# greatscottgadgets/libbtbb

Measured on AMD Instinct MI355X. Metric: Gbit/s raw bitstream scanned (LAP_ANY, err<=2), higher is better.
Workload: dtype u64; 1 GPU; promiscuous LAP_ANY scan, 4 GiB packed single-channel synthetic bitstream per GPU, max_ac_errors=2, sync word every 4096 symbols; symbols_per_gpu=34359738305, hits_per_gpu=6402406, parallelism=time-sharded x1 (btbbx_shard_plan: slices + 63-symbol halo), no collectives

## Files before the change

libbtbb_amd/csrc/packet.hip:

```cpp
#include <stdlib.h>
#include <string.h>
#include <atomic>
#include <type_traits>
#include "packet_launch.h"
#include "packet_core.h"

static uint32_t host_crc_byte(uint32_t crc, uint32_t byte)
{
	uint32_t x = (crc ^ byte) & 0xff;
	x ^= (x << 4) & 0xff;
	return ((crc >> 8) ^ (x << 8) ^ (x << 3) ^ (x >> 4)) & 0xffff;
}

int chain_upload(const HostTables &t)
{
	{
		int seen[16] = {0};
		for (int clk = 0; clk < 64; clk++) {
			uint32_t v = 0;
			for (int j = 0; j < 4; j++)
				v |= (uint32_t)t.whiten[(t.whiten_idx[clk] + 3 + j) % 127] << j;
			seen[v]++;
		}
		for (int v = 0; v < 16; v++)
// ... 197 lines not shown
{
	int rc = ctx_require();
	if (rc)
		return rc;
	hipLaunchKernelGGL(trials_state_kernel, dim3(64), dim3(64), 0, stream, d_sym, d_in, d_out, (TrialState *)d_state, d_trials);
	HIP_TRY(hipGetLastError());
	return BTBBX_OK;
}

int launch_trials_merge(const void *d_state, const btbbx_pkt_in *d_in, btbbx_pkt_out *d_out, uint8_t *d_pay,
			const TrialPlan *plan, hipStream_t stream)
{
	hipLaunchKernelGGL(trials_merge_kernel, dim3(1), dim3(64), 0, stream, (const TrialState *)d_state, d_in, d_out, d_pay,
			   *plan);
	HIP_TRY(hipGetLastError());
	return BTBBX_OK;
}

size_t trials_state_bytes() { return 64 * sizeof(TrialState); }

int launch_gather(const uint64_t *d_words, uint64_t n_words, uint64_t pitch_words, const btbbx_hit *d_hits, uint32_t n_packets,
		  const uint32_t *d_count, uint32_t max_length, uint64_t *d_packets, uint32_t *d_lengths, hipStream_t hip_stream)
{
	int rc = ctx_require();
	if (rc)
		return rc;
	if (!n_packets)
		return BTBBX_OK;
	hipLaunchKernelGGL(gather_kernel, dim3((n_packets + GATHER_PACKETS - 1) / GATHER_PACKETS), dim3(256), 0,
			   hip_stream, d_words, n_words, pitch_words, d_hits, n_packets, max_length, d_packets, d_lengths, d_count);
	HIP_TRY(hipGetLastError());
	return BTBBX_OK;
}

extern "C" int btbbx_gather_packets_device(const uint64_t *d_words, uint64_t n_words, uint64_t pitch_words,
					   const btbbx_hit *d_hits, uint32_t n_packets, uint32_t max_length,
					   uint64_t *d_packets, uint32_t *d_lengths, void *hip_stream)
{
	return launch_gather(d_words, n_words, pitch_words, d_hits, n_packets, nullptr, max_length, d_packets, d_lengths, (hipStream_t)hip_stream);
}

extern "C" int btbbx_trials_device(const uint64_t *d_packets, const btbbx_pkt_in *d_in, uint32_t n_packets,
				   btbbx_trial *d_trials, void *hip_stream)
{
	return launch_trials(d_packets, d_in, n_packets, nullptr, d_trials, (hipStream_t)hip_stream);
}

int launch_trials(const uint64_t *d_packets, const btbbx_pkt_in *d_in, uint32_t n_packets, const uint32_t *d_count,
		  btbbx_trial *d_trials, hipStream_t hip_stream)
{
	int rc = ctx_require();
	if (rc)
		return rc;
	if (!n_packets)
		return BTBBX_OK;
	if (n_packets <= 256) {
		hipLaunchKernelGGL(trials_wide_kernel, dim3(n_packets * 64), dim3(64), 0, (hipStream_t)hip_stream,
				   d_packets, d_in, n_packets, d_trials, d_count);
	} else {
		const uint32_t batches = (n_packets + TL_PACKETS - 1) / TL_PACKETS;
		const uint32_t resident = (uint32_t)ctx().num_cus * TL_WGS_PER_CU;
		hipLaunchKernelGGL(trials_linear_kernel, dim3(batches < resident ? batches : resident), dim3(TL_THREADS), 0,
				   (hipStream_t)hip_stream, d_packets, d_in, n_packets, d_trials, d_count);
	}
#ifdef TL_PROFILE
	if (n_packets > 256) {
		unsigned long long prof[16], tot = 0;
		(void)hipDeviceSynchronize();
		(void)hipMemcpyFromSymbol(prof, HIP_SYMBOL(g_tl_prof), sizeof(prof));
		for (int k = 0; k < 16; k++) tot += prof[k];
		fprintf(stderr, "trials profile:");
		for (int k = 0; k < 10; k++) fprintf(stderr, " %d:%.1f%%", k, 100.0 * (double)prof[k] / (double)(tot ? tot : 1));
		fprintf(stderr, "\n");
		static unsigned long long z[16];
		(void)hipMemcpyToSymbol(HIP_SYMBOL(g_tl_prof), z, sizeof(z));
	}
#endif
	HIP_TRY(hipGetLastError());
	return BTBBX_OK;
}

extern "C" int btbbx_uap_table_device(const uint64_t *d_packets, const btbbx_pkt_in *d_in, uint32_t n_packets,
				      uint16_t *d_table, void *hip_stream)
{
	int rc = ctx_require();
	if (rc)
		return rc;
	if (!n_packets)
		return BTBBX_OK;
	if ((uintptr_t)d_table & 15) {
		set_error("btbbx_uap_table_device: table must be 16-byte aligned");
		return BTBBX_E_ARG;
	}
	hipLaunchKernelGGL(uap_table_kernel, dim3((n_packets + 255) / 256), dim3(256), 0, (hipStream_t)hip_stream,
			   d_packets, d_in, n_packets, (uint4 *)d_table);
	HIP_TRY(hipGetLastError());
	return BTBBX_OK;
}

int launch_header_flags(const uint64_t *d_packets, const uint32_t *d_lengths, uint32_t n_packets, const uint32_t *d_count,
			uint8_t *d_present, hipStream_t stream)
{
	if (!n_packets)
		return BTBBX_OK;
	hipLaunchKernelGGL(header_flags_kernel, dim3((n_packets + 255) / 256), dim3(256), 0, stream, d_packets, d_lengths, n_packets, d_present, d_count);
	HIP_TRY(hipGetLastError());
	return BTBBX_OK;
}

int launch_decode_bytes(const uint8_t *d_sym, uint8_t *d_pay, const btbbx_pkt_in *d_in, btbbx_pkt_out *d_out,
			uint32_t mode, bool with_payload, hipStream_t stream)
{
	int rc = ctx_require();
	if (rc)
		return rc;
	hipLaunchKernelGGL(decode_bytes_kernel, dim3(1), dim3(64), 0, stream, d_sym, d_pay, d_in, d_out, mode,
			   with_payload ? 1 : 0);
	HIP_TRY(hipGetLastError());
	return BTBBX_OK;
}

int launch_decode(const uint64_t *d_packets, const btbbx_pkt_in *d_in, uint32_t n_packets,
		  btbbx_pkt_out *d_out, uint32_t mode, const TrialPlan *plan, hipStream_t stream)
{
	int rc = ctx_require();
	if (rc)
		return rc;
	if (!n_packets)
		return BTBBX_OK;
	TrialPlan p = {0, 0, 0};
	if (plan)
		p = *plan;
	if (mode & DEC_TRIALS) {
		if (mode != DEC_TRIALS || n_packets != 1) {
			set_error("decode: trial replay is a one-packet mode");
			return BTBBX_E_ARG;
		}
		hipLaunchKernelGGL(replay_kernel, dim3(1), dim3(64), 0, stream, d_packets, d_in, d_out, p);
		HIP_TRY(hipGetLastError());
		return BTBBX_OK;
	}
	hipLaunchKernelGGL(decode_kernel, dim3((n_packets + 63) / 64), dim3(64), 0, stream,
			   d_packets, d_in, n_packets, d_out, mode);
	HIP_TRY(hipGetLastError());
	return BTBBX_OK;
}

extern "C" int btbbx_decode_device(const uint64_t *d_packets, const btbbx_pkt_in *d_in, uint32_t n_packets,
				   btbbx_pkt_out *d_out, void *hip_stream)
{
	return launch_decode(d_packets, d_in, n_packets, d_out, DEC_HEADER | DEC_PAYLOAD, nullptr, (hipStream_t)hip_stream);
}

static int decode_hits_list_alloc(size_t bytes, hipStream_t stream, void **block)
{
	static std::atomic<uint64_t> pool_ready{0}, pool_absent{0};
	*block = nullptr;
	int dev = 0;
	HIP_TRY(hipGetDevice(&dev));
	const bool tracked = dev >= 0 && dev < 64;
	if (tracked && ((pool_absent.load() >> dev) & 1))
		return BTBBX_OK;
	if (tracked && !((pool_ready.load() >> dev) & 1)) {
		hipMemPool_t pool;
		uint64_t keep = UINT64_MAX;
		if (hipDeviceGetDefaultMemPool(&pool, dev) != hipSuccess ||
		    hipMemPoolSetAttribute(pool, hipMemPoolAttrReleaseThreshold, &keep) != hipSuccess) {
			(void)hipGetLastError();
			pool_absent.fetch_or(1ULL << dev);
			return BTBBX_OK;
		}
		pool_ready.fetch_or(1ULL << dev);
	}
	if (hipMallocAsync(block, bytes, stream) != hipSuccess) {
		(void)hipGetLastError();
		*block = nullptr;
	}
	return BTBBX_OK;
}

static int launch_decode_hits(const uint64_t *d_words, uint64_t n_words, uint64_t pitch_words, const btbbx_hit *d_hits,
			      const btbbx_pkt_in *d_in, uint32_t n_packets, const uint32_t *d_count, uint32_t max_length,
			      btbbx_pkt_out *d_out, uint32_t *d_lengths, const btbbx_pkt_in &one_in, uint32_t clk_div, hipStream_t stream)
{
	const uint32_t groups = (uint32_t)(((uint64_t)n_packets + 255) / 256);
	void *block;
	const int rc = decode_hits_list_alloc((size_t)groups * 4 * 64 * sizeof(uint4), stream, &block);
	if (rc)
		return rc;
	hipLaunchKernelGGL(decode_hits_kernel, dim3(groups), dim3(256), 0, stream, d_words, n_words, pitch_words, d_hits, d_in, n_packets,
			   d_count, max_length, d_out, d_lengths, DEC_HEADER | DEC_PAYLOAD, one_in, clk_div, (uint4 *)block);
	hipError_t e = hipGetLastError();
	if (block) {
		const hipError_t f = hipFreeAsync(block, stream);
		if (e == hipSuccess)
			e = f;
	}
	HIP_TRY(e);
	return BTBBX_OK;
}

extern "C" int btbbx_decode_hits_device(const uint64_t *d_words, uint64_t n_words, uint64_t pitch_words,
					const btbbx_hit *d_hits, const btbbx_pkt_in *d_in, uint32_t n_packets,
					uint32_t max_length, btbbx_pkt_out *d_out, uint32_t *d_lengths, void *hip_stream)
{
	int rc = ctx_require();
	if (rc)
		return rc;
	if (!n_packets)
		return BTBBX_OK;
	if (!d_words || !d_hits || !d_in || !d_out) {
		set_error("btbbx_decode_hits_device: null pointer");
		return BTBBX_E_ARG;
	}
	return launch_decode_hits(d_words, n_words, pitch_words, d_hits, d_in, n_packets, nullptr, max_length, d_out, d_lengths, btbbx_pkt_in{}, 1u,
				  (hipStream_t)hip_stream);
}

extern "C" int btbbx_decode_hits_counted_device(const uint64_t *d_words, uint64_t n_words, uint64_t pitch_words,
						const btbbx_hit *d_hits, const btbbx_pkt_in *d_in, const uint32_t *d_count,
						uint32_t cap, uint32_t max_length, btbbx_pkt_out *d_out, uint32_t *d_lengths,
						void *hip_stream)
{
	int rc = ctx_require();
	if (rc)
		return rc;
	if (!cap)
		return BTBBX_OK;
	if (!d_words || !d_hits || !d_in || !d_out || !d_count) {
		set_error("btbbx_decode_hits_counted_device: null pointer");
		return BTBBX_E_ARG;
	}
	rc = launch_decode_hits(d_words, n_words, pitch_words, d_hits, d_in, cap, d_count, max_length, d_out, d_lengths, btbbx_pkt_in{}, 1u,
				(hipStream_t)hip_stream);
	if (rc)
		return rc;
#ifdef DH_PROFILE
	{
		unsigned long long prof[8], total = 0;
		HIP_TRY(hipDeviceSynchronize());
		HIP_TRY(hipMemcpyFromSymbol(prof, HIP_SYMBOL(g_dh_prof), sizeof(prof)));
		for (int k = 0; k < 8; k++) total += prof[k];
		fprintf(stderr, "decode_hits profile (%% of wave time): loads %.1f type %.1f staging %.1f head-load %.1f present %.1f header %.1f payload %.1f store %.1f; s_memtime ticks per wave %.0f\n",
			100.0 * prof[0] / total, 100.0 * prof[1] / total, 100.0 * prof[2] / total, 100.0 * prof[3] / total,
			100.0 * prof[4] / total, 100.0 * prof[5] / total, 100.0 * prof[6] / total, 100.0 * prof[7] / total,
			(double)total / ((cap + 63) / 64));
		unsigned long long zero[8] = {0, 0, 0, 0, 0, 0, 0, 0};
		HIP_TRY(hipMemcpyToSymbol(HIP_SYMBOL(g_dh_prof), zero, sizeof(zero)));
	}
#endif
	return BTBBX_OK;
}

extern "C" int btbbx_decode_hits_piconet_phase_device(const uint64_t *d_words, uint64_t n_words, uint64_t pitch_words,
						      const btbbx_hit *d_hits, const uint32_t *d_count, uint32_t cap,
						      const btbbx_pkt_in *entry, uint32_t clk_div, uint32_t clk_phase, uint32_t max_length,
						      btbbx_pkt_out *d_out, uint32_t *d_lengths, void *hip_stream)
{
	int rc = ctx_require();
	if (rc)
		return rc;
	if (!cap)
		return BTBBX_OK;
	if (!d_words || !d_hits || !entry || !d_out || !clk_div || clk_phase >= clk_div) {
		set_error("btbbx_decode_hits_piconet_device: null pointer, clk_div = 0 or clk_phase >= clk_div");
		return BTBBX_E_ARG;
	}
	btbbx_pkt_in one = *entry;
	one.length = clk_phase;
	return launch_decode_hits(d_words, n_words, pitch_words, d_hits, nullptr, cap, d_count, max_length, d_out, d_lengths, one, clk_div,
				  (hipStream_t)hip_stream);
}

extern "C" int btbbx_decode_hits_piconet_device(const uint64_t *d_words, uint64_t n_words, uint64_t pitch_words,
						const btbbx_hit *d_hits, const uint32_t *d_count, uint32_t cap,
						const btbbx_pkt_in *entry, uint32_t clk_div, uint32_t max_length,
						btbbx_pkt_out *d_out, uint32_t *d_lengths, void *hip_stream)
{
	return btbbx_decode_hits_piconet_phase_device(d_words, n_words, pitch_words, d_hits, d_count, cap, entry, clk_div, 0, max_length,
						      d_out, d_lengths, hip_stream);
}
```

libbtbb_amd/csrc/packet_core.h:

```cpp
#pragma once
#include "defer_entry.h"

__constant__ ChainTables g_chain;

struct __attribute__((aligned(16))) ChainLds {
	uint32_t wh32[128];
	uint16_t crc[256];
	uint16_t crc_z[3][256];
	uint8_t  par23[1024];
	int8_t   fix23[32];
	uint16_t fixm23[32];
	uint8_t  whiten_idx[64];
	uint16_t adv32[2][256];
};
__device__ __attribute__((aligned(16))) ChainLds g_chain_lds_image;

#define LIN_MAXLEN 344
__device__ __attribute__((aligned(16))) uint16_t g_lin[LIN_MAXLEN * 16];
__device__ __attribute__((aligned(16))) uint16_t g_advw[7 * 2 * 256];
__device__ __attribute__((aligned(16))) uint16_t g_adv64inv[64 * 16];
__device__ __attribute__((aligned(16))) uint16_t g_adv64fwd[64 * 16];

#define F_WHITENED    (1u << 0)
#define F_CLK6_VALID  (1u << 4)
// ... 15 lines not shown
	const uint32_t *d = reinterpret_cast<const uint32_t *>(w);
	const uint32_t i = pos >> 5;
	const uint32_t v = __builtin_amdgcn_alignbit(d[i + 1], d[i], pos & 31);
	return n == 32 ? v : v & ((1u << n) - 1);
}

__device__ __forceinline__ uint64_t wh_bits_const(uint32_t idx, uint32_t n)
{
	uint32_t i = idx >> 6, s = idx & 63;
	uint64_t v = g_chain.whiten2[i] >> s;
	if (s + n > 64)
		v |= g_chain.whiten2[i + 1] << (64 - s);
	return n == 64 ? v : v & ((1ULL << n) - 1);
}

__device__ __forceinline__ uint32_t wh_start_const(uint32_t clock, uint32_t skip)
{
	return (g_chain.whiten_idx[clock & 63] + skip) % 127u;
}

__shared__ ChainLds g_lds;

__device__ __forceinline__ uint64_t wh_bits(uint32_t idx, uint32_t n)
{
	uint64_t v = g_lds.wh32[idx];
	if (n > 32) {
		const uint32_t j = idx + 32;
		v |= (uint64_t)g_lds.wh32[j >= 127 ? j - 127 : j] << 32;
	}
	return n == 64 ? v : v & ((1ULL << n) - 1);
}

__device__ __forceinline__ uint32_t wh_start(uint32_t clock, uint32_t skip)
{
	return (g_lds.whiten_idx[clock & 63] + skip) % 127u;
}

__device__ __forceinline__ uint32_t rev8(uint32_t b) { return __brev(b) >> 24; }

__device__ __forceinline__ uint32_t crc_byte_calc(uint32_t crc, uint32_t byte)
{
	uint32_t x = (crc ^ byte) & 0xff;
	x ^= (x << 4) & 0xff;
	return ((crc >> 8) ^ (x << 8) ^ (x << 3) ^ (x >> 4)) & 0xffff;
}
__device__ __forceinline__ uint32_t crc_byte(uint32_t crc, uint32_t byte)
{
	return (crc >> 8) ^ g_lds.crc[(crc ^ byte) & 0xff];
}

__device__ __forceinline__ uint32_t crc_word(uint32_t crc, uint32_t w)
{
	const uint32_t x = crc ^ w;
	return g_lds.crc_z[2][x & 0xff] ^ g_lds.crc_z[1][(x >> 8) & 0xff] ^ g_lds.crc_z[0][(w >> 16) & 0xff] ^ g_lds.crc[w >> 24];
}

__device__ __forceinline__ uint32_t crc_seed(uint32_t uap) { return rev8(uap & 0xff) << 8; }

__device__ __forceinline__ uint32_t uap_from_hec(uint32_t data, uint32_t hec)
{
#pragma unroll
	for (int i = 9; i >= 0; i--) {
		if (hec & 0x80)
			hec ^= 0x65;
		hec = ((hec << 1) | (((hec >> 7) ^ (data >> i)) & 1)) & 0xff;
	}
	return rev8(hec);
}

__device__ __forceinline__ uint32_t fec13(uint64_t v, uint32_t n, uint32_t &disagree)
{
	const uint64_t M = 0x9249249249249249ULL;
	uint64_t a = v & M, b = (v >> 1) & M, c = (v >> 2) & M;
	uint64_t maj = (a & b) | (b & c) | (c & a);
	uint64_t dis = (a ^ b) | (b ^ c) | (c ^ a);
	if (n < 21) {
		uint64_t keep = (1ULL << (3 * n)) - 1;
		maj &= keep;
		dis &= keep;
	}
	disagree = __popcll(dis);
	uint64_t x = maj;
	x = (x | x >> 2) & 0x30c30c30c30c30c3ULL;
	x = (x | x >> 4) & 0xf00f00f00f00f00fULL;
	x = (x | x >> 8) & 0x00ff0000ff0000ffULL;
	x = (x | x >> 16) & 0xffff00000000ffffULL;
	x = (x | x >> 32) & 0xffffffffULL;
	return (uint32_t)x;
}

__device__ __forceinline__ bool fec23_block(uint32_t blk, uint32_t &data)
{
	data = blk & 0x3ff;
	uint32_t diff = (blk >> 10) ^ g_lds.par23[data];
	int fix = g_lds.fix23[diff & 31];
	if (fix == -2)
		return false;
	if (fix >= 0)
		data ^= 1u << fix;
	return true;
}

__device__ void chain_lds_init()
{
	static_assert(sizeof(ChainLds) % 16 == 0, "the image is copied 16 bytes at a time");
	const uint4 *src = reinterpret_cast<const uint4 *>(&g_chain_lds_image);
	uint4 *dst = reinterpret_cast<uint4 *>(&g_lds);
	for (uint32_t i = threadIdx.x; i < sizeof(ChainLds) / 16; i += blockDim.x)
		dst[i] = src[i];
	__syncthreads();
}


struct OutRef {
	uint64_t *g = nullptr;
	uint32_t l = 0;
	__device__ OutRef() {}
	__device__ OutRef(uint64_t *p) : g(p) {}
	__device__ __forceinline__ static OutRef lds(uint32_t byte_address) { OutRef r; r.l = byte_address + 1; return r; }
	__device__ __forceinline__ uint64_t ld(uint32_t k) const
	{
		if (l)
			return *reinterpret_cast<const __attribute__((address_space(3))) uint64_t *>(l - 1 + 8u * k);
		return g[k];
	}
	__device__ __forceinline__ void st(uint32_t k, uint64_t v) const
	{
		if (l)
			*reinterpret_cast<__attribute__((address_space(3))) uint64_t *>(l - 1 + 8u * k) = v;
		else
			g[k] = v;
	}
};
struct PState {
	const uint64_t *w;
	uint32_t sh = 0;
	uint32_t wlimit = 0;
	uint32_t staged = 0;
	uint32_t stage_off = 0;
	bool direct = false;
	bool has_pre = false;
	uint32_t pre_hdr = 0, pre_dis = 0;
	int length;
	uint32_t flags;
	uint32_t uap, type;
	uint32_t lt_addr, hdr_flags, hec, header18;
	int plen;
	int phl;
	uint32_t ph16;
	uint32_t ph_written;
	uint32_t llid, flow;
	OutRef out;
	bool spoiled = false;
	uint4 *def_slot = nullptr;
	uint32_t def_pkt8 = 0;
	uint32_t def_nbits = 0;
	uint32_t written;
	uint32_t dirty;
	uint32_t ph_mask;
};
#define D_UT    1u
#define D_PLEN  2u
#define D_PHL   4u
#define D_LF    8u

__device__ __forceinline__ void pstate_enter(PState &s, const btbbx_pkt_in &pi)
{
	s.flags = pi.flags;
	s.uap = pi.uap;
	s.type = pi.type;
	s.llid = pi.llid;
	s.flow = pi.flow;
}
__device__ __forceinline__ void pstate_from_head(PState &s, int plen, int phl, uint32_t ph16, uint32_t lt_addr, uint32_t hdr_flags,
						 uint32_t hec, uint32_t header18)
{
	s.plen = plen;
	s.phl = phl;
	s.ph16 = ph16;
	s.ph_written = 0;
	s.dirty = 0;
	s.ph_mask = 0;
	s.lt_addr = lt_addr; s.hdr_flags = hdr_flags; s.hec = hec; s.header18 = header18;
	s.written = 0;
}
__device__ __forceinline__ void pstate_from_head(PState &s, const btbbx_pkt_out *o)
{
	pstate_from_head(s, o->payload_length, o->payload_header_length, (uint32_t)o->payload_header, o->lt_addr, o->hdr_flags, o->hec, o->header_packed);
}
__device__ __forceinline__ void pstate_blank_out(PState &s) { pstate_from_head(s, 0, 0, 0, 0, 0, 0, 0); }

__device__ __forceinline__ uint64_t s_bits(const PState &s, uint32_t pos, uint32_t n)
{
	if (!s.direct)
		return pk_bits(s.w, pos, n);
	if ((int)pos >= s.length)
		return 0;
	const uint32_t q = pos + s.sh, i = q >> 6, sft = q & 63;
	auto word = [&](uint32_t k) -> uint64_t {
		if (k < s.staged)
			return *reinterpret_cast<const __attribute__((address_space(3))) uint64_t *>(s.stage_off + 8u * k);
		return k < s.wlimit ? ((const __attribute__((address_space(1))) uint64_t *)(uintptr_t)s.w)[k] : 0ULL;
	};
	uint64_t v = word(i) >> sft;
	if (sft + n > 64)
		v |= word(i + 1) << (64 - sft);
	const uint32_t have = (uint32_t)s.length - pos;
	const uint32_t keep = n < have ? n : have;
	return keep == 64 ? v : v & ((1ULL << keep) - 1);
}

template <bool WRITE>
struct Sink {
	uint64_t acc = 0;
	uint32_t nacc = 0;
	uint32_t crc;
	uint64_t oacc = 0;
	uint32_t onacc = 0, oword = 0;
	OutRef out;
	__device__ Sink(uint32_t seed, OutRef o) : crc(seed), out(o) {}
	__device__ __forceinline__ void push(uint64_t bits, uint32_t n)
	{
		if (n == 32 && nacc == 0) {
			crc = crc_word(crc, (uint32_t)bits);
		} else {
			acc |= bits << nacc;
			nacc += n;
			while (nacc >= 8) {
				crc = crc_byte(crc, (uint32_t)acc & 0xff);
				acc >>= 8;
				nacc -= 8;
			}
		}
		if (WRITE) {
			oacc |= bits << onacc;
			onacc += n;
			if (onacc >= 64) {
				out.st(oword++, oacc);
				onacc -= 64;
				oacc = onacc ? bits >> (n - onacc) : 0;
			}
		}
	}
	__device__ __forceinline__ void flush()
	{
		if (WRITE && onacc) {
			uint64_t keep = ~0ULL << onacc;
			out.st(oword, (out.ld(oword) & keep) | oacc);
		}
	}
};

__device__ __forceinline__ bool whitened(const PState &s) { return s.flags & F_WHITENED; }

__device__ __forceinline__ uint64_t wh(const PState &s, uint32_t idx, uint32_t n)
{
	return whitened(s) ? wh_bits(idx, n) : 0ULL;
}

__device__ __forceinline__ uint32_t fec23_blocks4(const PState &s, uint32_t pos, uint32_t count, uint32_t (&data)[4])
{
	uint32_t blk[4], diff[4];
	const uint64_t sym60 = s_bits(s, pos, 60);
#pragma unroll
	for (int j = 0; j < 4; j++)
		blk[j] = (uint32_t)j < count ? (uint32_t)(sym60 >> (15 * j)) & 0x7fff : 0;
#pragma unroll
	for (int j = 0; j < 4; j++) {
		data[j] = blk[j] & 0x3ff;
		diff[j] = (blk[j] >> 10) ^ g_lds.par23[data[j]];
	}
	uint32_t ok = 0;
#pragma unroll
	for (int j = 0; j < 4; j++) {
		const int fix = g_lds.fix23[diff[j] & 31];
		if (fix >= 0)
			data[j] ^= 1u << fix;
		if (fix != -2)
			ok |= 1u << j;
	}
	return ok;
}

__device__ __forceinline__ bool fec23_ok(const PState &s, uint32_t pos, uint32_t nblocks)
{
	for (uint32_t k = 0; k < nblocks; k += 4) {
		uint32_t d[4];
		const uint32_t cnt = nblocks - k < 4 ? nblocks - k : 4;
		if ((fec23_blocks4(s, pos + 15 * k, cnt, d) & ((1u << cnt) - 1)) != (1u << cnt) - 1)
			return false;
	}
	return true;
}

__device__ __forceinline__ void defer_payload(PState &s, uint32_t clock, uint32_t nbits, uint32_t kind)
{
	const uint32_t ext = kind == DHL_DH ? nbits : kind == DHL_EV5 ? 8u : 15u * ((nbits + 9u) / 10u);
	const uint32_t nw = (s.sh + 122u + ext + 63u) >> 6;
	const uint64_t a = DEFER_PACK_A((uintptr_t)s.w, nw < s.wlimit ? nw : s.wlimit, s.sh);
	const uint64_t b = DEFER_PACK_B(s.def_pkt8, (uint32_t)s.length, nbits, kind, (s.flags & 1u) ? 1u : 0u, wh_start(clock, 18), s.uap & 0xffu);
	*s.def_slot = make_uint4((uint32_t)a, (uint32_t)(a >> 32), (uint32_t)b, (uint32_t)(b >> 32));
	s.def_nbits = nbits;
}

template <bool WRITE>
struct SinkW : Sink<WRITE> {
	__device__ SinkW(uint32_t seed, OutRef o) : Sink<WRITE>(seed, o) {}
	__device__ __forceinline__ void push(uint64_t bits, uint32_t n)
	{
		this->acc |= bits << this->nacc;
		this->nacc += n;
		if (this->nacc >= 32) {
			this->crc = crc_word(this->crc, (uint32_t)this->acc);
			this->acc >>= 32;
			this->nacc -= 32;
		}
		if (WRITE) {
			this->oacc |= bits << this->onacc;
			this->onacc += n;
			if (this->onacc >= 64) {
				this->out.st(this->oword++, this->oacc);
				this->onacc -= 64;
				this->oacc = this->onacc ? bits >> (n - this->onacc) : 0;
			}
		}
	}
	__device__ __forceinline__ void finish()
	{
		while (this->nacc >= 8) {
			this->crc = crc_byte(this->crc, (uint32_t)this->acc & 0xff);
			this->acc >>= 8;
			this->nacc -= 8;
		}
	}
};
template <bool WRITE>
__device__ __forceinline__ int do_fhs(PState &s, uint32_t clock)
{
	int size = s.length - 122;
	s.plen = 20;
	s.dirty |= D_PLEN;
	if (size < 240)
		return 1;
	uint64_t corr[3] = {0, 0, 0};
#pragma unroll
	for (uint32_t k = 0; k < 16; k += 4) {
		uint32_t d4[4];
		const uint32_t ok = fec23_blocks4(s, 122 + 15 * k, 4, d4);
#pragma unroll
		for (uint32_t j = 0; j < 4; j++) {
			if (!((ok >> j) & 1))
				return 0;
			const uint32_t d = d4[j], bit = 10 * (k + j);
			corr[bit >> 6] |= (uint64_t)d << (bit & 63);
			if ((bit & 63) > 54)
				corr[(bit >> 6) + 1] |= (uint64_t)d >> (64 - (bit & 63));
		}
	}
	int rv = 0;
	uint32_t c = clock;
	for (int attempt = 0; attempt < 33; attempt++) {
		if (attempt)
			c = 31 + attempt;
		uint32_t idx = wh_start(c, 18);
		uint32_t crc = crc_seed(s.uap);
		uint64_t pl[3];
		for (int i = 0; i < 3; i++) {
			uint32_t n = i < 2 ? 64 : 32;
			pl[i] = corr[i] ^ wh(s, idx, n);
			idx = (idx + n) % 127u;
			for (uint32_t b = 0; b < n; b += 32)
				crc = crc_word(crc, (uint32_t)(pl[i] >> b));
		}
		if (WRITE) {
			s.out.st(0, pl[0]);
			s.out.st(1, pl[1]);
			s.out.st(2, (s.out.ld(2) & ~0xffffffffULL) | pl[2]);
			if (s.written < 160) s.written = 160;
		}
		if (crc == 0) {
			rv = 1000;
			break;
		}
	}
	return rv;
}

template <bool WRITE>
__device__ __forceinline__ bool do_payload_header(PState &s, uint32_t pos, uint32_t clock, int header_bytes, int size, bool fec)
{
	uint32_t hbits = header_bytes == 2 ? 16 : 8;
	if (size < (int)hbits)
		return false;
	uint32_t raw;
	if (fec) {
		if (size < (header_bytes == 2 ? 30 : 15))
			return false;
		uint32_t d0, d1 = 0;
		if (!fec23_block((uint32_t)s_bits(s, pos, 15), d0))
			return false;
		if (header_bytes == 2 && !fec23_block((uint32_t)s_bits(s, pos + 15, 15), d1))
			return false;
		raw = (d0 | (d1 << 10)) & ((1u << hbits) - 1);
	} else {
		raw = (uint32_t)s_bits(s, pos, hbits);
	}
	uint32_t ph = raw ^ (uint32_t)wh(s, wh_start(clock, 18), hbits);
	s.ph16 = (s.ph16 & ~((1u << hbits) - 1)) | ph;
	s.ph_mask |= (1u << hbits) - 1;
	s.dirty |= D_PLEN | D_LF | D_PHL;
	if (s.ph_written < hbits) s.ph_written = hbits;
	int plen = header_bytes == 2 ? (int)((s.ph16 >> 3) & 0x3ff) + 4 : (int)((s.ph16 >> 3) & 0x1f) + 3;
	int cap;
	switch (s.type) {
	case 3:  cap = 20;  break;
	case 4:  cap = 30;  break;
	case 8:  cap = 12;  break;
	case 10: cap = 125; break;
	case 11: cap = 187; break;
	case 14: cap = 228; break;
	case 15: cap = 343; break;
	default: cap = 0;   break;
	}
	s.plen = plen < cap ? plen : cap;
	s.llid = s.ph16 & 3;
	s.flow = (s.ph16 >> 2) & 1;
	s.phl = header_bytes;
	return true;
}

template <bool WRITE>
__device__ __forceinline__ int do_DM(PState &s, uint32_t clock)
{
	uint32_t pos = 122;
	int size = s.length - 122;
	int header_bytes = 2, max_length;
	switch (s.type) {
	case 8:  pos += 80; size -= 80; header_bytes = 1; max_length = 12; break;
	case 3:  header_bytes = 1; max_length = 20; break;
	case 10: max_length = 125; break;
	case 14: max_length = 228; break;
	default: return 0;
	}
	if (!do_payload_header<WRITE>(s, pos, clock, header_bytes, size, true))
		return 0;
	if (s.plen > max_length)
		return 1;
	int nbits = s.plen * 8;
	if (nbits > size)
		return 1;
	uint32_t nblocks = (nbits + 9) / 10;
	if (WRITE && s.def_slot && !s.out.l && nbits > DHL_MIN_BITS) {
		defer_payload(s, clock, (uint32_t)nbits, DHL_DM);
		return 2;
// ... 274 lines not shown
```

libbtbb_amd/csrc/packet_stream.h:

```cpp
#pragma once


#ifdef DH_PROFILE
__device__ unsigned long long g_dh_prof[8];
#define DH_MARK(k) do { uint64_t now_; __builtin_amdgcn_sched_barrier(0); asm volatile("s_waitcnt vmcnt(0) lgkmcnt(0)\n\ts_memtime %0\n\ts_waitcnt lgkmcnt(0)" : "=s"(now_) : : "memory"); \
	__builtin_amdgcn_sched_barrier(0); dh_acc[k] += (uint32_t)(now_ - dh_t); dh_t = now_; } while (0)
#define DH_PARAMS , uint32_t *dh_acc, uint64_t &dh_t
#define DH_PASS , dh_acc, dh_t
#else
#define DH_MARK(k) do { } while (0)
#define DH_PARAMS
#define DH_PASS
#endif
__device__ __forceinline__ void decode_view(PState &s, const btbbx_pkt_in &pi, btbbx_pkt_out *o, uint32_t mode,
					    OutRef pay_out, uint64_t *head_out, const uint64_t *head_in DH_PARAMS)
{
	pstate_enter(s, pi);
	static_assert(offsetof(btbbx_pkt_out, payload) == 40 && offsetof(btbbx_pkt_out, payload_header) == 32, "head of btbbx_pkt_out");
	union Head {
		uint64_t q[5];
		struct {
			int32_t header_rv, payload_rv, payload_length, payload_header_length;
			uint32_t flags, header_packed;
			uint8_t header_present, type, lt_addr, hdr_flags, hec, llid, flow, uap;
// ... 509 lines not shown
					w0 = src[i0];
				if (i1 < p_nw)
					w1 = src[i1];
			}
		}
	};
	uint64_t nw0, nw1;
	request(0, nw0, nw1);
#pragma unroll 1
	for (uint32_t r = 0; r < rounds; r++) {
		const uint32_t e = r * R + grp;
		const bool has = e < n_ev;
		uint64_t pa = 0, pb = 0;
		if (has) {
			pa = lst[DHL_LIST + 2 * (first + e)];
			pb = lst[DHL_LIST + 2 * (first + e) + 1];
		}
		const uint32_t p_sh = DEFER_SH(pa);
		const uint32_t p_pkt = DEFER_PKT(pb), nbits = DEFER_NBITS(pb);
		const uint32_t kind = DEFER_KIND(pb), p_widx = DEFER_WIDX(pb), p_uap = DEFER_UAP(pb);
		const bool p_wht = DEFER_WHITENED(pb), is4 = has && kind == DHL_EV4;
		const uint32_t nblocks = nbits / 10u;
		const uint64_t w0 = nw0, w1 = nw1;
		const uint32_t sft = (p_sh + 122u) & 63u;
		const uint32_t low8 = (uint32_t)(sft ? (w0 >> sft) | (w1 << (64u - sft)) : w0) & 0xffu;
		const uint32_t first8 = (uint32_t)__shfl((int)low8, (int)gbase);
		uint64_t word = (uint64_t)(first8 * 0x01010101u) | (uint64_t)(first8 * 0x01010101u) << 32;
		uint32_t first_fail = nblocks;
		if (__ballot(is4)) {
			stg[2 * gbase + sub] = w0;
			stg[2 * gbase + G + sub] = w1;
			__builtin_amdgcn_fence(__ATOMIC_ACQ_REL, "wavefront");
			__builtin_amdgcn_wave_barrier();
			for (uint32_t n0 = 0; ; n0 += G) {
				const uint32_t n = n0 + sub;
				const bool on = is4 && 4u * n < nblocks;
				if (!__ballot(on))
					break;
				const uint32_t left = nblocks - 4u * n, have = on ? (left < 4u ? left : 4u) : 0u;
				const uint32_t q = p_sh + 122u + 60u * n, i = 4u * gbase + (on ? q >> 5 : 0u);
				const uint32_t v0 = stg32[i], v1 = stg32[i + 1], v2 = stg32[i + 2];
				const uint64_t vm = (1ULL << (15u * have)) - 1;
				const uint32_t x0 = __builtin_amdgcn_alignbit(v1, v0, q & 31u) & (uint32_t)vm;
				const uint32_t x1 = __builtin_amdgcn_alignbit(v2, v1, q & 31u) & (uint32_t)(vm >> 32);
				const uint32_t b2 = __builtin_amdgcn_alignbit(x1, x0, 30);
				uint32_t d0 = x0 & 0x3ffu, d1 = (x0 >> 15) & 0x3ffu, d2 = b2 & 0x3ffu, d3 = (x1 >> 13) & 0x3ffu;
				const uint32_t m0 = g_lds.fixm23[((x0 >> 10) & 31u) ^ g_lds.par23[d0]], m1 = g_lds.fixm23[((x0 >> 25) & 31u) ^ g_lds.par23[d1]];
				const uint32_t m2 = g_lds.fixm23[((b2 >> 10) & 31u) ^ g_lds.par23[d2]], m3 = g_lds.fixm23[((x1 >> 23) & 31u) ^ g_lds.par23[d3]];
				const uint32_t bad = (m0 >> 15) | (m1 >> 15) << 1 | (m2 >> 15) << 2 | (m3 >> 15) << 3;
				d0 ^= m0 & 0x3ffu;
				d1 ^= m1 & 0x3ffu;
				d2 ^= m2 & 0x3ffu;
				d3 ^= m3 & 0x3ffu;
				if (on) {
					const uint32_t byte = 5u * n, d = 2u * DHL_PB + 2u * gbase + (byte >> 2);
					const uint64_t v = ((uint64_t)(d3 >> 2) << 32 | (d0 | d1 << 10 | d2 << 20 | d3 << 30)) << (8u * (byte & 3u));
					__hip_atomic_fetch_or(lst32 + d, (uint32_t)v, __ATOMIC_RELAXED, __HIP_MEMORY_SCOPE_WAVEFRONT);
					__hip_atomic_fetch_or(lst32 + d + 1, (uint32_t)(v >> 32), __ATOMIC_RELAXED, __HIP_MEMORY_SCOPE_WAVEFRONT);
				}
				const uint64_t gm = (__ballot(bad != 0) >> gbase) & gmask;
				const uint32_t gl = gm ? (uint32_t)__builtin_ctzll(gm) : 0u;
				const uint32_t gb = (uint32_t)__shfl((int)bad, (int)(gbase + gl));
				if (gm && first_fail == nblocks)
					first_fail = 4u * (n0 + gl) + (uint32_t)__builtin_ctz(gb | 16u);
			}
			__builtin_amdgcn_fence(__ATOMIC_ACQ_REL, "wavefront");
			__builtin_amdgcn_wave_barrier();
			if (is4)
				word = lst[DHL_PB + lane];
			lst[DHL_PB + lane] = 0;
		}
		if (r + 1 < rounds)
			request(r + 1, nw0, nw1);
		const uint32_t T = nbits >> 6;
		const bool active = has && 64u * sub < nbits;
		uint64_t out = 0;
		if (active) {
			uint32_t idx = p_widx + wh_lane;
			idx = idx >= 127u ? idx - 127u : idx;
			out = word ^ (p_wht ? wh_bits(idx, 64) : 0ULL);
			if (sub == T)
				out &= (1ULL << (nbits & 63u)) - 1;
		}
		uint32_t reg;
		{
			const uint64_t cw = out ^ (sub == 0 ? (uint64_t)crc_seed(p_uap) : 0ULL);
			const uint32_t reg0 = crc_word(crc_word(0, (uint32_t)cw), (uint32_t)(cw >> 32));
			const uint32_t q = apply_columns(rinv, reg0);
			uint32_t x = q, t;
			t = (uint32_t)__builtin_amdgcn_mov_dpp((int)x, 0x111, 0xf, 0xf, true); x ^= sub >= 1 ? t : 0u;
			t = (uint32_t)__builtin_amdgcn_mov_dpp((int)x, 0x112, 0xf, 0xf, true); x ^= sub >= 2 ? t : 0u;
			t = (uint32_t)__builtin_amdgcn_mov_dpp((int)x, 0x114, 0xf, 0xf, true); x ^= sub >= 4 ? t : 0u;
			if (logg > 3) {
				t = (uint32_t)__builtin_amdgcn_mov_dpp((int)x, 0x118, 0xf, 0xf, true); x ^= sub >= 8 ? t : 0u;
			}
			if (logg > 4) {
				t = (uint32_t)__shfl((int)x, (int)(gbase + 15));
				x ^= sub >= 16 ? t : 0u;
			}
			reg = apply_columns(rfwd, x ^ q);
		}
		const uint32_t ok_blocks = first_fail < nblocks ? first_fail : nblocks;
		const uint32_t hi = is4 ? (ok_blocks ? 5u * (ok_blocks - 1u) / 4u : 0u) : (nbits >> 3) - 1u, lo = is4 ? 2u : 3u;
		uint32_t zero = 0;
#pragma unroll
		for (int i = 0; i < 8; i++) {
			uint32_t byte = (uint32_t)(out >> (8 * i)) & 0xffu;
			if (i == 1 && sub == 0)
				byte ^= crc_seed(p_uap) >> 8;
			reg = crc_byte(reg, byte);
			const uint32_t L = 8u * sub + (uint32_t)i + 1u;
			if (reg == 0 && L >= lo && L <= hi)
				zero |= 1u << i;
		}
		const uint64_t hm = (__ballot(has && zero != 0) >> gbase) & gmask;
		const uint32_t hl = hm ? (uint32_t)__builtin_ctzll(hm) : 0u;
		const uint32_t hz = (uint32_t)__shfl((int)zero, (int)(gbase + hl));
		const uint32_t L_hit = hm ? 8u * hl + (uint32_t)__builtin_ctz(hz | 0x100u) + 1u : 0u;
		if (has) {
			uint32_t plen, wbits;
			int rv;
			if (is4) {
				if (L_hit) {
					rv = 10; plen = L_hit; wbits = 10u * ((8u * L_hit + 9u) / 10u + 1u);
				} else {
					plen = hi + 1u; wbits = 10u * ok_blocks;
					rv = ok_blocks == 98u ? 2 : first_fail < nblocks && first_fail < 3u ? 0 : 1;
				}
			} else {
				const uint32_t bytes = nbits >> 3;
				if (L_hit) {
					rv = 10; plen = L_hit; wbits = 8u * (L_hit + 1u);
				} else {
					plen = bytes; wbits = nbits; rv = bytes == 182u ? 2 : 1;
				}
			}
			const uint32_t wT = wbits >> 6, wrem = wbits & 63u;
			if (64u * sub < wbits) {
				uint64_t v = out;
				if (sub == wT) {
					const uint64_t wm = (1ULL << wrem) - 1;
					v = (out & wm) | (outs[p_pkt].payload[sub] & ~wm);
				}
				outs[p_pkt].payload[sub] = v;
			}
			if (sub == 0) {
				outs[p_pkt].payload_length = (int32_t)plen;
				outs[p_pkt].payload_rv = rv;
			}
		}
	}
}

__device__ __forceinline__ void long_wave(dhl_u64_t *stg, dhl_u64_t *lst, const uint4 *slots, uint64_t dmask, btbbx_pkt_out *outs, uint32_t lane)
{
	const bool mine = (dmask >> lane) & 1;
	uint4 e = make_uint4(0, 0, 0, 0);
	if (mine)
		e = slots[lane];
	const bool ev = mine && DEFER_KIND_HI(e.w) >= DHL_EV4;
	const uint64_t ev_mask = __ballot(ev), dh_mask = dmask & ~ev_mask;
	const uint32_t n_dh = (uint32_t)__popcll(dh_mask), n_ev = (uint32_t)__popcll(ev_mask);
	const uint32_t own_words = mine ? (DEFER_NBITS_LO(e.z) + 63u) >> 6 : 0u;
	if (mine) {
		const uint64_t among = ev ? ev_mask : dh_mask;
		const uint32_t rank = (ev ? n_dh : 0u) + __builtin_amdgcn_mbcnt_hi((uint32_t)(among >> 32), __builtin_amdgcn_mbcnt_lo((uint32_t)among, 0u));
		lst[DHL_LIST + 2 * rank] = (uint64_t)e.x | (uint64_t)e.y << 32;
		lst[DHL_LIST + 2 * rank + 1] = (uint64_t)e.z | (uint64_t)e.w << 32;
	}
	if (n_dh) {
		const uint32_t w = ev ? 0u : own_words;
		if (__ballot(mine && !ev && DEFER_KIND_HI(e.w) == DHL_DM)) {
			const uint32_t logg = __ballot(w > 32) ? 5u : __ballot(w > 16) ? 4u : 3u;
			long_payloads(stg, lst, n_dh, logg, outs, lane);
		} else {
			dh_payloads(lst, n_dh, __ballot(w > 24) ? 4u : 3u, outs, lane);
		}
	}
	if (n_ev) {
		const uint32_t w = ev ? own_words : 0u;
		const uint32_t logg = __ballot(w > 16) ? 5u : __ballot(w > 8) ? 4u : 3u;
		ev_payloads(stg, lst, n_dh, n_ev, logg, outs, lane);
	}
}

#define DH_WAVES_PER_EU 6
__global__ __launch_bounds__(256) __attribute__((amdgpu_waves_per_eu(DH_WAVES_PER_EU, DH_WAVES_PER_EU)))
void decode_hits_kernel(const uint64_t *words, uint64_t n_words, uint64_t pitch_words,
							  const btbbx_hit *hits, const btbbx_pkt_in *in, uint32_t n_packets,
							  const uint32_t *d_count, uint32_t max_length, btbbx_pkt_out *outs,
							  uint32_t *lengths, uint32_t mode, btbbx_pkt_in one_in, uint32_t clk_div,
							  uint4 *long_list)
{
	__shared__ uint64_t stage[4][DH_STAGE_WORDS];
	__shared__ uint64_t ostage[4][64 * DH_OUT_WORDS];
	chain_lds_init();
	uint32_t pkt = blockIdx.x * blockDim.x + threadIdx.x;
	const uint32_t lane = threadIdx.x & 63, wave = threadIdx.x >> 6;
	if (d_count)
		n_packets = min(n_packets, *d_count);
	bool live = pkt < n_packets;
	if (blockIdx.x * blockDim.x >= n_packets)
		return;
#ifdef DH_PROFILE
	uint32_t dh_acc[8] = {0, 0, 0, 0, 0, 0, 0, 0};
	uint64_t dh_t;
	asm volatile("s_memtime %0\n\ts_waitcnt lgkmcnt(0)" : "=s"(dh_t) : : "memory");
#endif
	btbbx_hit h;
	h.offset = 0;
	h.stream = 0;
	if (live)
		h = hits[pkt];
	const uint64_t total_bits = n_words * 64;
	const uint64_t avail = h.offset < total_bits ? total_bits - h.offset : 0;
	uint32_t len = avail < max_length ? (uint32_t)avail : max_length;
	if (len > BTBBX_MAX_SYMBOLS)
		len = BTBBX_MAX_SYMBOLS;
	const uint64_t first_word = h.offset >> 6;
	PState s;
	s.w = words + (uint64_t)h.stream * pitch_words + first_word;
	s.sh = (uint32_t)(h.offset & 63);
	s.wlimit = first_word < n_words ? (uint32_t)(n_words - first_word < 64 ? n_words - first_word : 64) : 0;
	s.direct = true;
	s.length = live ? (int)len : 0;
	btbbx_pkt_in pi;
	pi.length = 0; pi.clkn = 0; pi.flags = 0; pi.uap = 0; pi.type = 0; pi.llid = 0; pi.flow = 0;
	if (live) {
		if (in) {
			pi = in[pkt];
		} else {
			pi = one_in;
			const uint64_t since = h.offset + one_in.length;
			pi.clkn = one_in.clkn + (since >> 32 ? (uint32_t)(since / clk_div) : (uint32_t)since / clk_div);
		}
	}
	pi.length = len;

	asm volatile("" : "+v"(pi.clkn), "+v"(len));
	DH_MARK(0);
	uint32_t want = 0, dtype = 0;
	bool small = false, wide = false;
	uint32_t hdr = 0, dis = 0;
	typedef __attribute__((address_space(3))) uint64_t lds_u64_t;
	{
		uint64_t hw[4];
#pragma unroll
		for (uint32_t k = 0; k < 4; k++)
			hw[k] = live && k + 1 < s.wlimit ? s.w[k + 1] : 0ULL;
#pragma unroll
		for (uint32_t k = 0; k < 4; k++)
			stage[wave][lane * 5 + k + 1] = hw[k];
		s.staged = s.wlimit < 5 ? s.wlimit : 5;
		s.stage_off = (uint32_t)(uintptr_t)(lds_u64_t *)(&stage[wave][lane * 5]);
	}
	if (live) {
		want = len < 126 ? len : 126;
		s.flags = pi.flags;
		hdr = header_fec13(s, dis);
		if ((mode & DEC_PAYLOAD) && len > 126) {
			uint32_t type = pi.type;
			if (mode & DEC_HEADER)
				type = ((hdr ^ (uint32_t)wh(s, wh_start(pi.clkn, 0), 18)) >> 3) & 0xf;
			const uint32_t bound = payload_extent(s, type, pi.clkn, small, wide);
			want = len < bound ? len : bound;
			dtype = type;
		}
	}
	asm volatile("" : "+v"(want));
	s.staged = 0;
	if (live && lengths)
		lengths[pkt] = len;
	{
		uint32_t *const sort_cnt = reinterpret_cast<uint32_t *>(&ostage[0][0]);
		uint8_t *const perm = reinterpret_cast<uint8_t *>(&ostage[0][32]);
		uint64_t *const xch = &stage[0][0];
		const uint32_t tid = threadIdx.x;
		if (tid < 64)
			sort_cnt[tid] = 0;
		__syncthreads();
		uint32_t key = 63;
		if (live) {
			const uint32_t cls = want <= 126 ? 0 : decoder_of_type(dtype);
			const uint32_t lb = want <= 126 ? 0 : (want - 122) >> 5;
			key = cls * 8 + (lb < 7 ? lb : 7);
			if (!small && want > 126 && (cls == 2 || cls == 3)) {
				const uint32_t pbits = cls == 2 ? (want - 122) / 15 * 10 : want - 122, words = (pbits + 63) >> 6;
				key = cls == 2 ? 32u + (words > 32 ? 2u : words > 16 ? 1u : 0u)
					       : 1u + (words > 24 ? 1u : 0u);
			}
		}
		const uint32_t r = atomicAdd(&sort_cnt[key], 1u);
		xch[tid] = h.offset;
		xch[256 + tid] = (uint64_t)h.stream | (uint64_t)want << 16 | (uint64_t)wide << 28 | (uint64_t)small << 30 | (uint64_t)live << 31 | (uint64_t)pi.clkn << 32;
		xch[512 + tid] = (uint64_t)pi.flags | (uint64_t)pi.uap << 32 | (uint64_t)pi.type << 40 | (uint64_t)pi.llid << 48 | (uint64_t)pi.flow << 56;
		xch[768 + tid] = (uint64_t)hdr | (uint64_t)dtype << 24 | (uint64_t)dis << 32;
		__syncthreads();
		uint32_t c = sort_cnt[lane], incl = c;
		for (int d = 1; d < 64; d <<= 1) {
			const uint32_t u = __shfl_up(incl, d);
			if (lane >= (uint32_t)d)
				incl += u;
		}
		perm[__shfl(incl - c, key) + r] = (uint8_t)tid;
		__syncthreads();
		const uint32_t q = perm[tid];
		const uint64_t x0 = xch[q], x1 = xch[256 + q], x2 = xch[512 + q], x3 = xch[768 + q];
		__syncthreads();
		pkt = blockIdx.x * blockDim.x + q;
		h.offset = x0;
		h.stream = (uint16_t)x1;
		want = (uint32_t)(x1 >> 16) & 0xfff;
		wide = (x1 >> 28) & 1;
		small = (x1 >> 30) & 1;
		live = (x1 >> 31) & 1;
		pi.clkn = (uint32_t)(x1 >> 32);
		pi.flags = (uint32_t)x2;
		pi.uap = (uint8_t)(x2 >> 32); pi.type = (uint8_t)(x2 >> 40); pi.llid = (uint8_t)(x2 >> 48); pi.flow = (uint8_t)(x2 >> 56);
		const uint64_t avail2 = h.offset < total_bits ? total_bits - h.offset : 0;
		len = avail2 < max_length ? (uint32_t)avail2 : max_length;
		if (len > BTBBX_MAX_SYMBOLS)
			len = BTBBX_MAX_SYMBOLS;
		const uint64_t fw = h.offset >> 6;
		s.w = words + (uint64_t)h.stream * pitch_words + fw;
		s.sh = (uint32_t)(h.offset & 63);
		s.wlimit = fw < n_words ? (uint32_t)(n_words - fw < 64 ? n_words - fw : 64) : 0;
		s.length = live ? (int)len : 0;
		pi.length = len;
		hdr = (uint32_t)x3 & 0x3ffffu;
		dtype = (uint32_t)(x3 >> 24) & 0xfu;
		dis = (uint32_t)(x3 >> 32);
	}
	s.has_pre = true;
	s.pre_hdr = hdr;
	s.pre_dis = dis;
	DH_MARK(1);
	const uint64_t small_mask = __ballot(small), wide_mask = __ballot(wide), live_mask = __ballot(live);
	uint64_t head_in[5] = {0, 0, 0, 0, 0};
	if (live) {
#pragma unroll
		for (int k = 0; k < 5; k++)
			head_in[k] = reinterpret_cast<const uint64_t *>(outs + pkt)[k];
	}
	uint32_t nw = live ? (s.sh + want + 63) / 64 : 0;
	if (nw > s.wlimit)
		nw = s.wlimit;
	if (live && !small && want > 126 && nw > 4 && (decoder_of_type(dtype) == 2 || decoder_of_type(dtype) == 3))
		nw = 4;
	uint32_t before = nw;
	for (int d = 1; d < 64; d <<= 1) {
		const uint32_t t = __shfl_up(before, d);
		if (lane >= (uint32_t)d)
			before += t;
	}
	before -= nw;
	if (before + nw > DH_STAGE_WORDS)
		nw = 0;
	const uint32_t stage_base = (uint32_t)(uintptr_t)(lds_u64_t *)(&stage[wave][0]);
	typedef __attribute__((address_space(3))) uint32_t lds_u32_t;
	typedef __attribute__((address_space(1))) const uint32_t glb_u32_t;
	{
		lds_u32_t *const obase = (lds_u32_t *)(lds_u64_t *)(&ostage[wave][0]);
#pragma unroll
		for (uint32_t t = 0; t < 2 * DH_OUT_WORDS; t++) {
			const uint32_t f = t * 64 + lane, p = f / (2 * DH_OUT_WORDS), k = f % (2 * DH_OUT_WORDS);
			const uint32_t pkt_p = __shfl(pkt, p);
			if (((small_mask >> p) & 1) && (k < 2 * DH_OUT_SECTOR || ((wide_mask >> p) & 1)))
				__builtin_amdgcn_global_load_lds((glb_u32_t *)(uintptr_t)(reinterpret_cast<const uint32_t *>(outs + pkt_p) + 10 + k),
								 obase + t * 64, 4, 0, 0);
		}
	}
	{
		lds_u32_t *const sbase = (lds_u32_t *)(lds_u64_t *)(&stage[wave][0]);
		const uint64_t staged_mask = __ballot(nw > 0);
		const uint32_t last = staged_mask ? 63u - (uint32_t)__builtin_clzll(staged_mask) : 0u;
		const uint32_t total2 = staged_mask ? 2u * (uint32_t)__builtin_amdgcn_readlane(before + nw, last) : 0u;
		for (uint32_t k = 0; __ballot(k < nw); k++)
			if (k < nw)
				sbase[2 * (before + k)] = lane;
		const uint64_t adj = (uint64_t)(uintptr_t)s.w - 8ull * before;
		for (uint32_t d0 = 0; d0 < total2; d0 += 64) {
			const uint32_t d = d0 + lane;
			const uint32_t owner = d < total2 ? sbase[d & ~1u] : 0u;
			const uint64_t a = __shfl(adj, owner) + 4ull * d;
			if (d < total2)
				__builtin_amdgcn_global_load_lds((glb_u32_t *)(uintptr_t)a, sbase + d0, 4, 0, 0);
		}
	}
	asm volatile("s_waitcnt vmcnt(0)" : : : "memory");
	__builtin_amdgcn_wave_barrier();
	s.staged = nw;
	s.stage_off = stage_base + 8u * before;
	DH_MARK(2);

	uint64_t head[5] = {0, 0, 0, 0, 0};
	if (long_list) {
		s.def_slot = long_list + ((size_t)(blockIdx.x * 4 + wave) * 64 + lane);
		s.def_pkt8 = pkt - blockIdx.x * blockDim.x;
	}
	if (live)
		decode_view(s, pi, outs + pkt, mode,
			    small ? OutRef::lds((uint32_t)(uintptr_t)(lds_u64_t *)(&ostage[wave][lane * DH_OUT_WORDS])) : OutRef(), head, head_in DH_PASS);
	__builtin_amdgcn_wave_barrier();
	const uint64_t long_mask = long_list ? __ballot(live && s.def_nbits != 0) : 0ULL;
	const uint64_t keep_mask = __ballot(small && !s.spoiled);
#pragma unroll
	for (int k = 0; k < 5; k++)
		stage[wave][lane * 5 + k] = head[k];
	__builtin_amdgcn_wave_barrier();
#pragma unroll
	for (uint32_t t = 0; t < 5 + DH_OUT_WORDS; t++) {
		const uint32_t f = t * 64 + lane, p = f / (5 + DH_OUT_WORDS), k = f % (5 + DH_OUT_WORDS);
		const uint32_t pkt_p = __shfl(pkt, p);
		if ((live_mask >> p) & 1) {
			uint64_t *dst = reinterpret_cast<uint64_t *>(outs + pkt_p);
			if (k < 5)
				dst[k] = stage[wave][p * 5 + k];
			else if (((keep_mask >> p) & 1) && (k - 5 < DH_OUT_SECTOR || ((wide_mask >> p) & 1)))
				dst[k] = ostage[wave][p * DH_OUT_WORDS + k - 5];
		}
	}
	DH_MARK(7);
	if (__builtin_expect(long_mask != 0, 0)) {
		asm volatile("s_waitcnt vmcnt(0)" : : : "memory");
		__builtin_amdgcn_fence(__ATOMIC_ACQ_REL, "wavefront");
		__builtin_amdgcn_wave_barrier();
		uint32_t lane2 = __builtin_amdgcn_mbcnt_hi(~0u, __builtin_amdgcn_mbcnt_lo(~0u, 0u));
		asm volatile("" : "+v"(lane2));
		uint32_t wave2 = __builtin_amdgcn_readfirstlane(threadIdx.x >> 6);
		asm volatile("" : "+s"(wave2));
		long_wave((dhl_u64_t *)(lds_u64_t *)(&stage[wave2][0]), (dhl_u64_t *)(lds_u64_t *)(&ostage[wave2][0]), long_list + (size_t)(blockIdx.x * 4 + wave2) * 64, long_mask,
			  outs + (size_t)blockIdx.x * blockDim.x, lane2);
	}
#ifdef DH_PROFILE
	if (lane == 0)
		for (int k = 0; k < 8; k++)
			atomicAdd(&g_dh_prof[k], (unsigned long long)dh_acc[k]);
#endif
}
```

Baseline: 12840 Gbit/s.

## Keep deferred long-payload descriptors in LDS instead of a global scratch list

Deferred long-payload descriptors were written to a global buffer obtained per launch with hipMallocAsync/hipFreeAsync and read back in long_wave. They now go into the lane's own ostage LDS slot, packed as two 64-bit words. This drops the per-launch pool allocation and free, the global write and read round trip, and the vmcnt wait before the long-payload pass. The risk is that the descriptor shares LDS with the lane's output staging area and could clash with small-packet output data; the deferred path also becomes unconditional where it used to be skipped when the allocation failed.

```diff
diff --git a/libbtbb_amd/csrc/packet.hip b/libbtbb_amd/csrc/packet.hip
--- a/libbtbb_amd/csrc/packet.hip
+++ b/libbtbb_amd/csrc/packet.hip
@@ -373,50 +373,14 @@
 	return launch_decode(d_packets, d_in, n_packets, d_out, DEC_HEADER | DEC_PAYLOAD, nullptr, (hipStream_t)hip_stream);
 }
 
-static int decode_hits_list_alloc(size_t bytes, hipStream_t stream, void **block)
-{
-	static std::atomic<uint64_t> pool_ready{0}, pool_absent{0};
-	*block = nullptr;
-	int dev = 0;
-	HIP_TRY(hipGetDevice(&dev));
-	const bool tracked = dev >= 0 && dev < 64;
-	if (tracked && ((pool_absent.load() >> dev) & 1))
-		return BTBBX_OK;
-	if (tracked && !((pool_ready.load() >> dev) & 1)) {
-		hipMemPool_t pool;
-		uint64_t keep = UINT64_MAX;
-		if (hipDeviceGetDefaultMemPool(&pool, dev) != hipSuccess ||
-		    hipMemPoolSetAttribute(pool, hipMemPoolAttrReleaseThreshold, &keep) != hipSuccess) {
-			(void)hipGetLastError();
-			pool_absent.fetch_or(1ULL << dev);
-			return BTBBX_OK;
-		}
-		pool_ready.fetch_or(1ULL << dev);
-	}
-	if (hipMallocAsync(block, bytes, stream) != hipSuccess) {
-		(void)hipGetLastError();
-		*block = nullptr;
-	}
-	return BTBBX_OK;
-}
-
 static int launch_decode_hits(const uint64_t *d_words, uint64_t n_words, uint64_t pitch_words, const btbbx_hit *d_hits,
 			      const btbbx_pkt_in *d_in, uint32_t n_packets, const uint32_t *d_count, uint32_t max_length,
 			      btbbx_pkt_out *d_out, uint32_t *d_lengths, const btbbx_pkt_in &one_in, uint32_t clk_div, hipStream_t stream)
 {
 	const uint32_t groups = (uint32_t)(((uint64_t)n_packets + 255) / 256);
-	void *block;
-	const int rc = decode_hits_list_alloc((size_t)groups * 4 * 64 * sizeof(uint4), stream, &block);
-	if (rc)
-		return rc;
 	hipLaunchKernelGGL(decode_hits_kernel, dim3(groups), dim3(256), 0, stream, d_words, n_words, pitch_words, d_hits, d_in, n_packets,
-			   d_count, max_length, d_out, d_lengths, DEC_HEADER | DEC_PAYLOAD, one_in, clk_div, (uint4 *)block);
-	hipError_t e = hipGetLastError();
-	if (block) {
-		const hipError_t f = hipFreeAsync(block, stream);
-		if (e == hipSuccess)
-			e = f;
-	}
+			   d_count, max_length, d_out, d_lengths, DEC_HEADER | DEC_PAYLOAD, one_in, clk_div);
+	const hipError_t e = hipGetLastError();
 	HIP_TRY(e);
 	return BTBBX_OK;
 }
diff --git a/libbtbb_amd/csrc/packet_core.h b/libbtbb_amd/csrc/packet_core.h
--- a/libbtbb_amd/csrc/packet_core.h
+++ b/libbtbb_amd/csrc/packet_core.h
@@ -191,7 +191,7 @@
 	uint32_t llid, flow;
 	OutRef out;
 	bool spoiled = false;
-	uint4 *def_slot = nullptr;
+	uint32_t def_slot = 0;
 	uint32_t def_pkt8 = 0;
 	uint32_t def_nbits = 0;
 	uint32_t written;
@@ -338,7 +338,9 @@
 	const uint32_t nw = (s.sh + 122u + ext + 63u) >> 6;
 	const uint64_t a = DEFER_PACK_A((uintptr_t)s.w, nw < s.wlimit ? nw : s.wlimit, s.sh);
 	const uint64_t b = DEFER_PACK_B(s.def_pkt8, (uint32_t)s.length, nbits, kind, (s.flags & 1u) ? 1u : 0u, wh_start(clock, 18), s.uap & 0xffu);
-	*s.def_slot = make_uint4((uint32_t)a, (uint32_t)(a >> 32), (uint32_t)b, (uint32_t)(b >> 32));
+	__attribute__((address_space(3))) uint64_t *const slot = reinterpret_cast<__attribute__((address_space(3))) uint64_t *>(s.def_slot - 1);
+	slot[0] = a;
+	slot[1] = b;
 	s.def_nbits = nbits;
 }
 
diff --git a/libbtbb_amd/csrc/packet_stream.h b/libbtbb_amd/csrc/packet_stream.h
--- a/libbtbb_amd/csrc/packet_stream.h
+++ b/libbtbb_amd/csrc/packet_stream.h
@@ -685,12 +685,14 @@
 	}
 }
 
-__device__ __forceinline__ void long_wave(dhl_u64_t *stg, dhl_u64_t *lst, const uint4 *slots, uint64_t dmask, btbbx_pkt_out *outs, uint32_t lane)
+__device__ __forceinline__ void long_wave(dhl_u64_t *stg, dhl_u64_t *lst, uint64_t dmask, btbbx_pkt_out *outs, uint32_t lane)
 {
 	const bool mine = (dmask >> lane) & 1;
 	uint4 e = make_uint4(0, 0, 0, 0);
-	if (mine)
-		e = slots[lane];
+	if (mine) {
+		const uint64_t a = lst[DH_OUT_WORDS * lane], b = lst[DH_OUT_WORDS * lane + 1];
+		e = make_uint4((uint32_t)a, (uint32_t)(a >> 32), (uint32_t)b, (uint32_t)(b >> 32));
+	}
 	const bool ev = mine && DEFER_KIND_HI(e.w) >= DHL_EV4;
 	const uint64_t ev_mask = __ballot(ev), dh_mask = dmask & ~ev_mask;
 	const uint32_t n_dh = (uint32_t)__popcll(dh_mask), n_ev = (uint32_t)__popcll(ev_mask);
@@ -722,8 +724,7 @@
 void decode_hits_kernel(const uint64_t *words, uint64_t n_words, uint64_t pitch_words,
 							  const btbbx_hit *hits, const btbbx_pkt_in *in, uint32_t n_packets,
 							  const uint32_t *d_count, uint32_t max_length, btbbx_pkt_out *outs,
-							  uint32_t *lengths, uint32_t mode, btbbx_pkt_in one_in, uint32_t clk_div,
-							  uint4 *long_list)
+							  uint32_t *lengths, uint32_t mode, btbbx_pkt_in one_in, uint32_t clk_div)
 {
 	__shared__ uint64_t stage[4][DH_STAGE_WORDS];
 	__shared__ uint64_t ostage[4][64 * DH_OUT_WORDS];
@@ -927,15 +928,13 @@
 	DH_MARK(2);
 
 	uint64_t head[5] = {0, 0, 0, 0, 0};
-	if (long_list) {
-		s.def_slot = long_list + ((size_t)(blockIdx.x * 4 + wave) * 64 + lane);
-		s.def_pkt8 = pkt - blockIdx.x * blockDim.x;
-	}
+	s.def_slot = (uint32_t)(uintptr_t)(lds_u64_t *)(&ostage[wave][lane * DH_OUT_WORDS]) + 1;
+	s.def_pkt8 = pkt - blockIdx.x * blockDim.x;
 	if (live)
 		decode_view(s, pi, outs + pkt, mode,
 			    small ? OutRef::lds((uint32_t)(uintptr_t)(lds_u64_t *)(&ostage[wave][lane * DH_OUT_WORDS])) : OutRef(), head, head_in DH_PASS);
 	__builtin_amdgcn_wave_barrier();
-	const uint64_t long_mask = long_list ? __ballot(live && s.def_nbits != 0) : 0ULL;
+	const uint64_t long_mask = __ballot(live && s.def_nbits != 0);
 	const uint64_t keep_mask = __ballot(small && !s.spoiled);
 #pragma unroll
 	for (int k = 0; k < 5; k++)
@@ -955,14 +954,13 @@
 	}
 	DH_MARK(7);
 	if (__builtin_expect(long_mask != 0, 0)) {
-		asm volatile("s_waitcnt vmcnt(0)" : : : "memory");
 		__builtin_amdgcn_fence(__ATOMIC_ACQ_REL, "wavefront");
 		__builtin_amdgcn_wave_barrier();
 		uint32_t lane2 = __builtin_amdgcn_mbcnt_hi(~0u, __builtin_amdgcn_mbcnt_lo(~0u, 0u));
 		asm volatile("" : "+v"(lane2));
 		uint32_t wave2 = __builtin_amdgcn_readfirstlane(threadIdx.x >> 6);
 		asm volatile("" : "+s"(wave2));
-		long_wave((dhl_u64_t *)(lds_u64_t *)(&stage[wave2][0]), (dhl_u64_t *)(lds_u64_t *)(&ostage[wave2][0]), long_list + (size_t)(blockIdx.x * 4 + wave2) * 64, long_mask,
+		long_wave((dhl_u64_t *)(lds_u64_t *)(&stage[wave2][0]), (dhl_u64_t *)(lds_u64_t *)(&ostage[wave2][0]), long_mask,
 			  outs + (size_t)blockIdx.x * blockDim.x, lane2);
 	}
 #ifdef DH_PROFILE
```

Result: no change. 12820 Gbit/s (median of 3 runs) (-0.2%).
